# liuQuan98/GCL

Hardware: AMD Instinct MI355X
Metric: active voxels/sec thru ResUNetBN2C fwd+bwd+GCL loss, KITTI 0.3m (higher is better)
Workload: dtype f32; 1 GPU; configs[2]: GCL training step (finest_contrastive_loss), ResUNetBN2C-32 conv1 k=5, KITTI-shaped ray-cast clouds @0.3 m, bs=4 x 7 clouds per GPU, positive groups 'fixed16'; global_batch=4, parallelism=dp1

## Files before the change

gcl_amd/MinkowskiEngine/native.py:

```python
import ctypes
import os
import threading

import torch
from torch.autograd.function import once_differentiable

from .. import _lib

PLAN_ENABLED = os.environ.get("GCL_PLAN", "1") == "1"
AUX_STREAM = {"0": "", "1": "1", "low": "low", "high": "high"}[os.environ.get("GCL_PLAN_AUX", "low")]


def _addr(t):
    return t.data_ptr() if t is not None else 0


_SIDE_STREAMS = {}


def eval_side_stream(device, n_rows=None):
    if os.environ.get("GCL_EVAL_SPLIT_MAPS", "1") == "0":
        return None
    if n_rows is not None and n_rows < int(os.environ.get("GCL_EVAL_SPLIT_MIN_ROWS", "100000")):
        return None
# ... 66 lines not shown
            return None
        if addr == self.coords.data_ptr():
            return self.coords
        numel = 1
        for s in shape:
            numel *= int(s)
        nbytes = numel * torch.empty(0, dtype=dtype).element_size()
        off = addr - self.arena.data_ptr()
        if off < 0 or off + nbytes > self.arena.numel():
            raise RuntimeError("NativeMaps.view: address outside the arena")
        return self.arena[off:off + nbytes].view(dtype).view(*shape)


class _PlanRun:

    __slots__ = ("plan", "arena", "maps", "y", "x", "grad_targets", "segments", "done")

    def __del__(self):
        try:
            if not self.done and self.plan is not None and self.plan.handle and self.arena is not None:
                _lib.load().gcl_plan_release(self.plan.handle, ctypes.c_void_p(self.arena.data_ptr()))
        except Exception:
            pass


class _PlanFn(torch.autograd.Function):

    @staticmethod
    def forward(ctx, run, *params):
        ctx.run = run
        return run.y
# ... 31 lines not shown
            raise ValueError(lib.gcl_last_error().decode())
        self.handle = ctypes.c_void_p(self.handle)
        self._state = None
        self._key = None
        self.grad_targets = None
        self.bucket_of_param = None
        self.on_bucket = None
        self._param_ptrs = self._bn_ptrs = None
        self._ptr_key = None
        self.profile_next = False
        self.last_profile = None
        self._anchor = None
        self._aux = None
        self._eval_key = None
        self._touched = None

    def __del__(self):
        h, self.handle = getattr(self, "handle", None), None
        if h:
            try:
                _lib.load().gcl_plan_destroy(h)
            except Exception:
                pass

    @classmethod
    def from_tape(cls, tape, model, x_in, in_level, spec_keys):
        from . import ops
        if ops.PRECISION != "fp16x3" or not ops.FUSE_GRAD_ADD:
            raise ValueError("the plan runs the default arithmetic (fp16x3, fused gradient adds) only")
        params = [p for p in model.parameters()]
# ... 121 lines not shown
        self._ensure_state(lib, dev)
        pp, bp = self._pointers()
        if AUX_STREAM and self._aux is None:
            lo, _hi = torch.cuda.Stream.priority_range()
            pct = int(os.environ.get("GCL_AUX_CU_PCT", "0"))
            if 0 < pct < 100:
                h = ctypes.c_void_p()
                _lib.check(lib.gcl_stream_create_cu_share(pct, 1, ctypes.byref(h)), "gcl_stream_create_cu_share")
                self._aux = torch.cuda.ExternalStream(h.value, device=dev)
            else:
                self._aux = torch.cuda.Stream(device=dev, priority={"low": lo, "high": _hi}.get(AUX_STREAM, 0))
            lib.gcl_plan_set_aux_stream(self.handle, ctypes.c_void_p(self._aux.cuda_stream))
        if self.profile_next:
            lib.gcl_plan_profile(self.handle, 1)
        y_ptr = ctypes.c_void_p()
        _lib.check(lib.gcl_plan_forward(self.handle, ctypes.byref(maps.desc), _lib.ptr(x, torch.float32), pp, bp,
                                        _lib.ptr(self._state), _lib.ptr(arena), arena.numel(), ctypes.byref(y_ptr),
                                        _lib.stream()), "gcl_plan_forward")
        for m in self.bn_modules:
            m._pending_batches += 1
            m._train_forwards += 1
        n_out = int(maps.desc.n_rows[self.records[-1]["level_out"]])
        off = y_ptr.value - arena.data_ptr()
        y = arena[off:off + n_out * self.out_channels * 4].view(torch.float32).view(n_out, self.out_channels)
        if not torch.is_grad_enabled():
            lib.gcl_plan_release(self.handle, _lib.ptr(arena))
            return y
        run = _PlanRun()
        run.plan, run.arena, run.maps, run.y, run.x = self, arena, maps, y, x
        run.grad_targets, run.done = self.grad_targets, False
        run.segments = self._segments()
        if run.grad_targets is not None:
            if self._anchor is None or self._anchor.device != dev:
                self._anchor = torch.zeros(1, device=dev, requires_grad=True)
            return _PlanFn.apply(run, self._anchor)
        return _PlanFn.apply(run, *self.params)

    def _check_input(self, x_feats, maps):
        r0 = self.records[0]
        if x_feats.dim() != 2 or x_feats.shape[1] != r0["cin"]:
            raise ValueError(f"the plan was recorded for {r0['cin']} input channels, got a tensor of shape {tuple(x_feats.shape)}")
        if x_feats.shape[0] != int(maps.desc.n_rows[r0["level_in"]]):
            raise ValueError("features and coordinate maps differ in length")

    def _ensure_state(self, lib, dev):
# ... 51 lines not shown
        for i, r in enumerate(self.records):
            for k in ("w", "bias", "bn_w", "bn_b"):
                p = r[k]
                if p >= 0 and p in self.bucket_of_param:
                    b = self.bucket_of_param[p]
                    lowest[b] = min(lowest.get(b, i), i)
        cuts = sorted(set(lowest.values()), reverse=True)
        segs, hi = [], n
        for c in cuts:
            segs.append((c, hi, sorted(b for b, i in lowest.items() if i == c)))
            hi = c
        if hi > 0:
            segs.append((0, hi, []))
        return segs

    def set_touched_rows(self, rows, cap):
        lib = _lib.load()
        self._touched = rows
        _lib.check(lib.gcl_plan_set_touched_rows(self.handle, _lib.ptr(rows, torch.int32), int(cap)),
                   "gcl_plan_set_touched_rows")

    def touch_loss_rows(self, index, goff, sel, rows_a, rows_b, n_rows, cap):
        lib = _lib.load()
        dev = index.device
        scratch = torch.empty(int(lib.gcl_touched_rows_scratch_len(int(n_rows))), dtype=torch.int32, device=dev)
        out = torch.empty(int(cap) + 1, dtype=torch.int32, device=dev)
        rows, count = out[:cap], out[cap:]
        _lib.check(lib.gcl_touched_rows(_lib.ptr(index, torch.int64), index.shape[0], _lib.ptr(goff, torch.int64),
                                        goff.shape[0] - 1, _lib.ptr(sel, torch.int64), sel.shape[0],
                                        _lib.ptr(rows_a, torch.int64), rows_a.shape[0], _lib.ptr(rows_b, torch.int64),
                                        rows_b.shape[0], int(n_rows), _lib.ptr(scratch), _lib.ptr(rows), int(cap),
                                        _lib.ptr(count), _lib.stream()), "gcl_touched_rows")
        self.set_touched_rows(rows, cap)
# ... 5 lines not shown
        flat = None
        if targets is None:
            sizes = [p.numel() for p in self.params]
            flat = torch.empty(sum(sizes), dtype=torch.float32, device=dy.device)
            targets, off = [], 0
            for p, s in zip(self.params, sizes):
                targets.append(flat[off:off + s].view_as(p))
                off += s
        gp = (ctypes.c_void_p * len(targets))(*[t.data_ptr() for t in targets])
        st = _lib.stream()
        for first, last, buckets in run.segments:
            _lib.check(lib.gcl_plan_backward(self.handle, _lib.ptr(run.arena), _lib.ptr(dy, torch.float32), gp, first,
                                             last, st), "gcl_plan_backward")
            for b in buckets:
                self.on_bucket(b)
        self._touched = None
        if self.profile_next:
            self.profile_next = False
            self._profile_pending = True
            lib.gcl_plan_profile(self.handle, 0)
        run.done = True
        run.arena = run.maps = run.y = run.x = None
        return None if flat is None else targets

    def profile_records(self):
        lib = _lib.load()
        buf = (ctypes.c_double * (8 * 1024))()
        n = lib.gcl_plan_profile_read(self.handle, buf, 1024)
        return [tuple(buf[8 * i + j] for j in range(8)) for i in range(max(0, n))]
```

gcl_amd/_lib.py:

```python
import ctypes
import os
import subprocess

import torch

_HERE = os.path.dirname(os.path.abspath(__file__))
CSRC = os.path.join(_HERE, "csrc")
LIB_PATH = os.environ.get("GCL_LIB_PATH", os.path.join(CSRC, "libgcl_hip.so"))
SOURCES = ["coords.hip", "conv.hip", "norm.hip", "loss.hip", "pairloss.hip", "data.hip", "sc2pcr.hip", "plan.hip", "match.hip", "ransac.hip", "regstats.hip", "fpfh.hip",
           "valpose.hip", "pairmatch.hip", "icp.hip"]
HEADER = os.path.join(os.path.dirname(_HERE), "include", "gcl_amd.h")

_vp, _i32, _i64, _f32 = ctypes.c_void_p, ctypes.c_int32, ctypes.c_int64, ctypes.c_float
_f64 = ctypes.c_double

MAX_LEVELS, MAX_MAPS = 8, 16
MAPS_PINNED_BYTES = 512 * (MAX_MAPS + 1)
ERR_ARENA = -4


class MapSpec(ctypes.Structure):
    _fields_ = [("t_in", _i32), ("kernel_size", _i32), ("stride", _i32), ("tables", _i32), ("pairs", _i32)]


# ... 108 lines not shown
    "gcl_maps_build_split": (_i32, [_vp, _i64, _vp, _i32, _i32, _vp, _i64, _vp, _vp, _vp, _vp]),
    "gcl_plan_create": (_vp, [_vp, _i32, _i32, _i32, _vp, _i32, _i32]),
    "gcl_plan_destroy": (None, [_vp]),
    "gcl_plan_state_bytes": (_i64, [_vp]),
    "gcl_plan_arena_bytes": (_i64, [_vp, _vp]),
    "gcl_plan_forward": (_i32, [_vp, _vp, _vp, _vp, _vp, _vp, _vp, _i64, _vp, _vp]),
    "gcl_plan_eval_state_bytes": (_i64, [_vp]),
    "gcl_plan_eval_arena_bytes": (_i64, [_vp, _vp]),
    "gcl_plan_forward_eval": (_i32, [_vp, _vp, _vp, _vp, _vp, _i32, _vp, _vp, _i64, _vp, _vp]),
    "gcl_plan_backward": (_i32, [_vp, _vp, _vp, _vp, _i32, _i32, _vp]),
    "gcl_plan_release": (_i32, [_vp, _vp]),
    "gcl_plan_set_aux_stream": (_i32, [_vp, _vp]),
    "gcl_plan_touched_suffix": (_i32, [_vp]),
    "gcl_plan_set_touched_rows": (_i32, [_vp, _vp, _i64]),
    "gcl_plan_suffix_rows_used": (_i64, [_vp]),
    "gcl_gather_rows": (_i32, [_vp, _i32, _i64, _vp, _i64, _i32, _f32, _vp, _vp]),
    "gcl_scatter_rows": (_i32, [_vp, _vp, _i64, _i32, _i64, _vp, _i32, _vp]),
    "gcl_touched_rows_scratch_len": (_i64, [_i64]),
    "gcl_touched_rows": (_i32, [_vp, _i64, _vp, _i64, _vp, _i32, _vp, _i32, _vp, _i32, _i64, _vp, _vp, _i64, _vp, _vp]),
    "gcl_stream_create_cu_share": (_i32, [_i32, _i32, ctypes.POINTER(ctypes.c_void_p)]),
    "gcl_stream_destroy": (_i32, [_vp]),
    "gcl_plan_profile": (_i32, [_vp, _i32]),
    "gcl_plan_profile_read": (_i32, [_vp, _vp, _i32]),
    "gcl_sc2_chunks": (_i32, []),
    "gcl_sc2_refine_partial_len": (_i32, []),
    "gcl_sc2_confidence": (_i32, [_vp, _vp, _i32, _f32, _i32, _vp, _vp, _vp, _vp]),
    "gcl_sc2_confidence_scratch_bytes": (_i64, [_i32]),
    "gcl_sc2_confidence_sparse": (_i32, [_vp, _vp, _i32, _f32, _i32, _vp, _vp, _vp, _vp, _vp]),
    "gcl_sc2_register_scratch_bytes": (_i64, [_i32]),
    "gcl_sc2_register": (_i32, [_vp, _vp, _i32, _f32, _i32, _f32, _i32, _i32, _i32, _f32, _f32, _i32, _vp, _vp, _vp, _vp, _vp,
# ... 167 lines not shown
```

gcl_amd/csrc/plan.hip:

```cpp
#include "common.h"

#include <string.h>

#include <new>
#include <utility>
#include <vector>

namespace gcl {

__device__ __forceinline__ float amax4p(float m, const float4& v) {
  return fmaxf(m, fmaxf(fmaxf(fabsf(v.x), fabsf(v.y)), fmaxf(fabsf(v.z), fabsf(v.w))));
}
__device__ __forceinline__ void publish_amax_wg(float m, int* slot) {
#pragma unroll
  for (int o = 32; o > 0; o >>= 1) m = fmaxf(m, __shfl_xor(m, o));
  __shared__ float wm[4];
  if ((threadIdx.x & 63) == 0) wm[threadIdx.x >> 6] = m;
  __syncthreads();
  if (threadIdx.x == 0)
    amax_slot_publish(slot, __float_as_int(fmaxf(fmaxf(wm[0], wm[1]), fmaxf(wm[2], wm[3]))), blockIdx.x);
}

__global__ void __launch_bounds__(256) k_relu_fwd(const float4* __restrict__ x, long long n4, float4* __restrict__ y,
                                                  int* amax) {
// ... 94 lines not shown
    const long long j = i / cv;
    const int q = (int)(i - j * cv);
    const long long r = rows[j];
    out[i] = (r >= 0 && r < n_src) ? reinterpret_cast<const V*>(src + r * ld)[q] : splat<V>(pad);
  }
}
__global__ void __launch_bounds__(256) k_scatter_rows(const float4* __restrict__ src, const int* __restrict__ rows,
                                                      long long cap, int c4, long long n_dst, float* __restrict__ dst,
                                                      int ld) {
  const long long total = cap * c4;
  for (long long i = (long long)blockIdx.x * 256 + threadIdx.x; i < total; i += (long long)gridDim.x * 256) {
    const long long j = i / c4;
    const int q = (int)(i - j * c4);
    const long long r = rows[j];
    if (r >= 0 && r < n_dst) reinterpret_cast<float4*>(dst + r * ld)[q] = src[i];
  }
}
__global__ void __launch_bounds__(256) k_touch_rows(const long long* __restrict__ ids, long long count, long long n,
                                                    int* __restrict__ flag) {
  const long long i = (long long)blockIdx.x * 256 + threadIdx.x;
  if (i >= count) return;
  const long long r = ids[i];
  if (r >= 0 && r < n) flag[r] = 1;
}
__global__ void __launch_bounds__(64) k_touch_groups(const long long* __restrict__ index, long long n_index,
                                                     const long long* __restrict__ goff, long long n_groups,
                                                     const long long* __restrict__ sel, long long n,
                                                     int* __restrict__ flag) {
  const long long g = sel[blockIdx.x];
  if (g < 0 || g >= n_groups) return;
// ... 290 lines not shown
  std::vector<OpSaved> saved;
  std::vector<void*> params;
  Arena A{DRY_BASE, 0, 0, true};
  int32_t* slot_pool = nullptr;
  long long n_slots = 0, next_slot = 0;
  bool slots_exhausted = false;
  int32_t* w_amax = nullptr;
  unsigned char *pack_fwd = nullptr, *pack_bwd = nullptr;
  void* state = nullptr;
  bool forward_done = false, bwd_packed = false;
  std::vector<char> relu_masked;
  hipEvent_t fwd_packs = nullptr;
  bool fwd_packs_pending = false;
  int32_t* not_ones = nullptr;
  void* key = nullptr;
};

struct Plan : PassState {
  std::vector<PassState*> passes;
  std::vector<gcl_plan_op> ops;
  int n_tensors = 0, n_params = 0, n_bn = 0, presplit = 128;
  std::vector<int> worder;
  std::vector<int> widx;
  std::vector<int> wmode;
  std::vector<long long> wK, wcin, wcout, off_fwd, off_bwd;
  long long bytes_fwd = 0, bytes_bwd = 0, wgs_fwd = 0, wgs_bwd = 0;
  int n_bwd = 0;
  std::vector<char> made;
  std::vector<char> fuse_relu;
  std::vector<int> cat_left;
  std::vector<int> mask_from;
  std::vector<long long> host_tables, uploaded;
  bool eval = false;
  void* const* bn_eval = nullptr;
  bool eval_repack = true;
  hipStream_t aux = nullptr;
  std::vector<hipEvent_t> events;
  size_t events_used = 0;
  bool aux_dirty = false;
  int suffix_first = 0;
  bool suffix_rows_ok = false;
  const int32_t* touched = nullptr;
  long long touched_cap = 0;
  long long suffix_rows_used = 0;
  bool profile = false;
  std::vector<ProfRec> prof;
  size_t prof_used = 0;
};

static long long state_words(const Plan& P) { return (long long)P.worder.size() * (2 + 8 + 8); }

static int32_t* new_slot(Plan& P) {
  if (P.next_slot >= P.n_slots) {
    P.slots_exhausted = true;
    return P.slot_pool;
  }
  return P.slot_pool + (P.next_slot++) * GCL_AMAX_WORDS;
}

// ... 61 lines not shown

static bool is_stem(const gcl_plan_op& op, const gcl_map_desc& m) {
  return op.cin <= 4 && (op.cout % 32) == 0 && !op.transpose && m.kernel_size > 1 && op.bias < 0;
}

static int stem_flag(Plan& P, const gcl_plan_op& op, const gcl_map_desc& m, const TState& x, long long n_in, hipStream_t st) {
  Arena& A = P.A;
  if (!m.presence || P.not_ones) return GCL_OK;
  constexpr int CLOUD_FLAGS = 4096;
  int32_t* cloud = A.take_n<int32_t>(CLOUD_FLAGS);
  P.not_ones = A.take_n<int32_t>(n_in);
  PLAN_CALL(gcl_not_ones_rows(x.ptr, op.cin, P.maps->coords[op.level_in], n_in, cloud, CLOUD_FLAGS, P.not_ones, (void*)st));
  return GCL_OK;
}

static int conv_forward(Plan& P, int i, float** y_out, float** stats_out, hipStream_t st, int32_t** relu_amax_out) {
  Arena& A = P.A;
  const gcl_plan_op& op = P.ops[i];
  const gcl_maps_desc& M = *P.maps;
  const gcl_map_desc& m = M.maps[op.map];
  const long long n_in = M.n_rows[op.level_in], n_out = M.n_rows[op.level_out];
  TState& x = P.t[op.x];
  float* y = A.take_n<float>(n_out * op.cout);
  *y_out = y;
  *stats_out = nullptr;
  *relu_amax_out = nullptr;
  const float* W = (const float*)P.params[op.w];
  if (is_stem(op, m)) {
    int rcs = stem_flag(P, op, m, x, n_in, st);
    if (rcs) return rcs;
    PLAN_CALL(gcl_stem_fwd(x.ptr, W, m.nbr, n_out, op.K, op.cin, op.cout, y, m.presence, m.presence ? P.not_ones : nullptr,
                           (void*)st));
    return GCL_OK;
  }
  const int wi = P.widx[op.w];
  if (P.fwd_packs_pending && !A.dry) {
// ... 103 lines not shown
  }
  if (!P.eval && P.aux && P.n_bwd) {
    P.pack_bwd = (unsigned char*)A.take(P.bytes_bwd);
    if (!A.dry) {
      hipStream_t ws = fork_aux(P, st);
      const long long* tab = (const long long*)P.state;
      PLAN_CALL(gcl_pack_weights_multi((const int64_t*)(tab + 2 * nw + 8 * nw), P.n_bwd, P.wgs_bwd, 4, P.w_amax, P.pack_bwd,
                                       (void*)ws));
    }
    P.bwd_packed = true;
  }
  P.t[0].ptr = (float*)x_in;
  bool late_pending = !A.dry && M.ready_event && M.late_mask;
  for (size_t i = 0; i < P.ops.size(); ++i) {
    const gcl_plan_op& op = P.ops[i];
    const long long n_out = M.n_rows[op.level_out];
    if (late_pending && (op.kind == GCL_OP_CONVBN || op.kind == GCL_OP_CONV) && ((M.late_mask >> op.map) & 1)) {
      GCL_CHECK_HIP(hipStreamWaitEvent(st, (hipEvent_t)M.ready_event, 0));
      late_pending = false;
    }
    TState& y = P.t[op.y];
    int rc;
    switch (op.kind) {
      case GCL_OP_CONVBN: {
        if (P.eval) {
          const gcl_map_desc& m = M.maps[op.map];
          const long long n_in = M.n_rows[op.level_in];
          TState& x = P.t[op.x];
          const int c = op.cout;
          const float* res = op.x2 >= 0 ? P.t[op.x2].ptr : nullptr;
          y.ptr = A.take_n<float>(n_out * c);
// ... 69 lines not shown
          y.ld = 0;
          y.amax = bound ? bound_slot : new_slot(P);
          if (bound) y.planes = A.take(n_out * c * 4);
        }
        if (op.relu) sv.mask = A.take_n<unsigned long long>(gcl_bn_mask_len(n_out, c));
        const float* res = op.x2 >= 0 ? P.t[op.x2].ptr : nullptr;
        void* img = !bound ? nullptr : (P.cat_left[i] >= 0 ? P.t[P.ops[P.cat_left[i]].y].planes : y.planes);
        PLAN_CALL(gcl_bn_apply_planes(cy, n_out, c, sv.mean, sv.rstd, (const float*)P.params[op.bn_w],
                                      (const float*)P.params[op.bn_b], res, op.relu, y.ptr, y.ld, (uint64_t*)sv.mask, y.amax,
                                      img, (void*)st));
        break;
      }
      case GCL_OP_CONV: {
        float *cy, *stats;
        int32_t* relu_amax;
        if ((rc = conv_forward(P, (int)i, &cy, &stats, st, &relu_amax))) return rc;
        y.ptr = cy;
        if (relu_amax) {
          y.amax = relu_amax;
          P.t[P.ops[i + 1].y] = y;
        }
        break;
      }
      case GCL_OP_RELU: {
        if (i > 0 && P.fuse_relu[i - 1]) break;
        const long long n4 = n_out * op.cout / 4;
        y.ptr = A.take_n<float>(n_out * op.cout);
        y.amax = new_slot(P);
        if (!A.dry) {
          hipLaunchKernelGGL(k_relu_fwd, dim3(grid_for(n4)), dim3(256), 0, st, (const float4*)P.t[op.x].ptr, n4, (float4*)y.ptr,
                             y.amax);
          GCL_CHECK_LAUNCH();
        }
        break;
      }
      case GCL_OP_CAT: {
        const int ca = op.cin, cb = op.cout - op.cin;
        if (P.t[op.x].ld == op.cout && P.t[op.x].ptr == y.ptr && y.ptr) {
          if (!A.dry) {
            hipLaunchKernelGGL(k_cat_right, dim3(grid_for(n_out * cb / 4)), dim3(256), 0, st, (const float4*)P.t[op.x2].ptr,
// ... 15 lines not shown
        break;
      }
      case GCL_OP_ROWNORM: {
        y.ptr = A.take_n<float>(n_out * op.cout);
        P.saved[i].norm = A.take_n<float>(n_out);
        PLAN_CALL(gcl_row_normalize_fwd(P.t[op.x].ptr, n_out, op.cout, y.ptr, P.saved[i].norm, (void*)st));
        break;
      }
      default:
        set_error("gcl_plan_forward: unknown record kind %d", op.kind);
        return GCL_ERR_ARG;
    }
  }
  if (late_pending) GCL_CHECK_HIP(hipStreamWaitEvent(st, (hipEvent_t)M.ready_event, 0));
  *y_out = P.t[P.ops.back().y].ptr;
  return GCL_OK;
}

static int give(Plan& P, int tensor, float* gptr, long long numel, hipStream_t st, int32_t* amax = nullptr, int ld = 0,
                int c = 0) {
  Arena& A = P.A;
  if (tensor < 0 || !P.made[tensor] || !gptr) return GCL_OK;
  TState& g = P.g[tensor];
  if (!g.ptr) {
    g = TState();
    g.ptr = gptr;
    g.ld = ld;
    g.amax = amax;
    return GCL_OK;
  }
// ... 113 lines not shown
                                     dy.amax, scratch, dW, rgb, (void*)ws));
  }
  if (op.bias >= 0) {
    double* scratch = A.take_n<double>(gcl_bn_scratch_len(n_out, op.cout));
    PLAN_CALL(gcl_col_sum(dy.ptr, n_out, op.cout, scratch, (float*)grads[op.bias], (void*)ws));
  }
  return GCL_OK;
}

static int suffix_backward(Plan& P, const float* dy, void* const* grads, const int32_t* rows, long long cap, TState* g_out,
                           hipStream_t st) {
  Arena& A = P.A;
  const gcl_maps_desc& M = *P.maps;
  const int n_ops = (int)P.ops.size();
  const long long n = M.n_rows[P.ops.back().level_out];
  std::vector<std::pair<const float*, float*>> gathered;
  auto gather = [&](const float* src, int ld, int c, float pad) -> float* {
    for (auto& e : gathered)
      if (e.first == src) return e.second;
    float* out = A.take_n<float>(cap * c);
    if (!A.dry && gcl_gather_rows(src, ld, n, rows, cap, c, pad, out, (void*)st) != GCL_OK) return nullptr;
    gathered.push_back({src, out});
    return out;
  };
  std::vector<char> masked(P.ops.size(), 0);
  TState g;
  g.ptr = gather(dy, P.ops.back().cout, P.ops.back().cout, 0.f);
  if (!g.ptr) return GCL_ERR_ARG;
  int rc;
  for (int i = n_ops - 1; i >= P.suffix_first && g.ptr; --i) {
    const gcl_plan_op& op = P.ops[i];
    switch (op.kind) {
// ... 90 lines not shown
    P.pack_bwd = (unsigned char*)A.take(P.bytes_bwd);
    if (P.n_bwd && !A.dry) {
      const long long* tab = (const long long*)P.state;
      PLAN_CALL(gcl_pack_weights_multi((const int64_t*)(tab + 2 * nw + 8 * nw), P.n_bwd, P.wgs_bwd, 4, P.w_amax, P.pack_bwd,
                                       (void*)st));
    }
    P.bwd_packed = true;
  }
  int top = last - 1;
  long long reserve_to = 0;
  if (last == n_ops && !A.dry) P.suffix_rows_used = 0;
  if (last == n_ops && P.suffix_first < n_ops && P.suffix_rows_ok && first <= P.suffix_first) {
    const gcl_plan_op& head = P.ops[P.suffix_first];
    const long long n = M.n_rows[head.level_in];
    const long long off0 = A.off, slot0 = P.next_slot;
    if (A.dry) {
      TState g;
      const long long cap_max = (n - 1) / 2;
      if (cap_max > 0) {
        int rc = suffix_backward(P, dy, grads, nullptr, cap_max, &g, st);
        if (rc) return rc;
        A.take_n<float>(n * head.cin);
        reserve_to = A.off;
        A.off = off0;
        P.next_slot = slot0;
      }
    } else if (rows && cap > 0 && 2 * cap < n) {
      TState g;
      A.dry = true;
      int rc = suffix_backward(P, dy, grads, rows, cap, &g, st);
      A.take_n<float>(n * head.cin);
// ... 345 lines not shown
    std::vector<void*> gn(P->n_params, nullptr);
    float* yy = nullptr;
    const bool prof = P->profile;
    P->profile = false;
    rc = plan_forward(*P, x, bn_stats_host, &yy, nullptr);
    if (rc == GCL_OK) rc = plan_backward(*P, (const float*)DRY_BASE, gn.data(), 0, (int)P->ops.size(), nullptr);
    P->profile = prof;
    const long long need = P->A.off;
    P->A = real;
    if (rc) return rc;
    if (need > arena_bytes) {
      set_error("gcl_plan_forward: arena too small (%lld bytes needed, %lld given)", need, (long long)arena_bytes);
      return GCL_ERR_ARENA;
    }
  }
  rc = plan_forward(*P, x, bn_stats_host, y_out_host, (hipStream_t)stream);
  P->forward_done = rc == GCL_OK;
  if (rc != GCL_OK) return rc;
  PassState* slot = nullptr;
  for (PassState* q : P->passes)
    if (!q->forward_done || q->key == arena) slot = q;
  if (!slot) {
    slot = new (std::nothrow) PassState();
    GCL_CHECK_ARG(slot, "gcl_plan_forward: out of host memory");
    P->passes.push_back(slot);
  }
  P->key = arena;
  *slot = std::move(static_cast<PassState&>(*P));
  slot->maps = &slot->maps_copy;
  static_cast<PassState&>(*P) = PassState();
  return GCL_OK;
}

// ... 84 lines not shown
int gcl_plan_backward(void* plan, void* arena, const float* dy, void* const* grads_host, int32_t first_op,
                      int32_t last_op, void* stream) {
  Plan* P = (Plan*)plan;
  GCL_CHECK_ARG(P, "gcl_plan_backward: null pointer");
  const int32_t* rows = P->touched;
  const long long cap = P->touched_cap;
  P->touched = nullptr;
  P->touched_cap = 0;
  GCL_CHECK_ARG(grads_host, "gcl_plan_backward: null pointer");
  PassState* slot = nullptr;
  for (PassState* q : P->passes)
    if (q->forward_done && q->key == arena) slot = q;
  GCL_CHECK_ARG(slot, "gcl_plan_backward: no forward pass to differentiate in this arena");
  GCL_CHECK_ARG(first_op >= 0 && first_op < last_op && last_op <= (int)P->ops.size(), "gcl_plan_backward: bad record range");
  GCL_CHECK_ARG(last_op != (int)P->ops.size() || dy, "gcl_plan_backward: the last segment needs dy");
  static_cast<PassState&>(*P) = std::move(*slot);
  P->maps = &P->maps_copy;
  int rc = plan_backward(*P, dy, grads_host, first_op, last_op, (hipStream_t)stream, rows, cap);
  if (rc == GCL_OK && !P->A.fits()) {
    set_error("gcl_plan_backward: arena overrun");
    rc = GCL_ERR_ARENA;
  }
  if (rc == GCL_OK && P->slots_exhausted) {
    set_error("gcl_plan_backward: amax slot pool exhausted");
    rc = GCL_ERR_ARG;
  }
  if (first_op == 0 || rc != GCL_OK) P->forward_done = false;
  *slot = std::move(static_cast<PassState&>(*P));
  slot->maps = &slot->maps_copy;
  static_cast<PassState&>(*P) = PassState();
// ... 28 lines not shown

int gcl_scatter_rows(const float* src, const int32_t* rows, int64_t cap, int32_t c, int64_t n_dst, float* dst, int32_t ld,
                     void* stream) {
  GCL_CHECK_ARG(src && rows && dst && n_dst > 0 && cap > 0, "gcl_scatter_rows: bad argument");
  GCL_CHECK_ARG(c > 0 && c % 4 == 0 && ld >= c && ld % 4 == 0 && (((uintptr_t)src | (uintptr_t)dst) & 15) == 0,
                "gcl_scatter_rows: channel count and row pitch must be multiples of 4, the tensors 16-byte aligned");
  hipLaunchKernelGGL(k_scatter_rows, dim3(grid_for(cap * c / 4)), dim3(256), 0, (hipStream_t)stream, (const float4*)src,
                     (const int*)rows, (long long)cap, c / 4, (long long)n_dst, dst, ld);
  GCL_CHECK_LAUNCH();
  return GCL_OK;
}

int64_t gcl_plan_suffix_rows_used(const void* plan) {
  if (!plan) return -1;
  return ((const Plan*)plan)->suffix_rows_used;
}

int gcl_plan_set_touched_rows(void* plan, const int32_t* rows, int64_t cap) {
  Plan* P = (Plan*)plan;
  GCL_CHECK_ARG(P, "gcl_plan_set_touched_rows: null plan");
  GCL_CHECK_ARG((rows && cap > 0) || (!rows && cap == 0), "gcl_plan_set_touched_rows: a list needs a positive length");
  P->touched = rows;
  P->touched_cap = cap;
  return GCL_OK;
}

int64_t gcl_touched_rows_scratch_len(int64_t n_rows) { return n_rows > 0 ? gcl_scan_scratch_len(n_rows) : 0; }

int gcl_touched_rows(const int64_t* index, int64_t n_index, const int64_t* goff, int64_t n_groups, const int64_t* sel,
                     int32_t n_sel, const int64_t* rows_a, int32_t n_a, const int64_t* rows_b, int32_t n_b, int64_t n_rows,
// ... 74 lines not shown
```

gcl_amd/lib/colocation_trainer.py:

```python
import os
import types

import numpy as np
import torch
from torch.autograd.function import once_differentiable

import gcl_amd.MinkowskiEngine as ME
from gcl_amd import _lib
from gcl_amd.model import load_model

DEFAULT_CONFIG = dict(
    model="ResUNetBN2C", model_n_out=32, conv1_kernel_size=5, normalize_feature=True, bn_momentum=0.05,
    optimizer="SGD", lr=0.1, momentum=0.8, weight_decay=1e-4, exp_gamma=0.99,
    batch_size=4, num_pos_per_batch=256, num_hn_samples_per_batch=256, iter_size=1,
    hit_ratio_thresh=0.3, val_max_iter=400, nn_max_n=500,
    pos_thresh=0.1, neg_thresh=1.4, finest_thresh=0.2, pos_weight=1.0, neg_weight=1.0, finest_weight=1.0,
    square_loss=True, block_finest_gradient=False, use_hard_negative=True, use_pair_group_positive_loss=False,
    use_group_circle_loss=False, safe_radius=0.75, voxel_size=0.3,
    triplet_num_pos=256, triplet_num_hn=512, triplet_num_rand=1024,
)


def make_config(**overrides):
    cfg = dict(DEFAULT_CONFIG)
# ... 150 lines not shown


def prepare_loss_inputs(group, index, finest_flag, device):
    group = torch.as_tensor(group)
    goff = torch.zeros(int(group.shape[0]) + 1, dtype=torch.int64, device=device)
    goff[1:] = torch.cumsum(group.to(device, torch.int64, non_blocking=True), 0)
    index = torch.as_tensor(index).to(device, torch.int64, non_blocking=True).contiguous()
    flag = torch.as_tensor(finest_flag).to(device, non_blocking=True).to(torch.uint8).contiguous()
    return goff, index, flag


def finest_contrastive_loss(F_out, group, index, index_hash, finest_flag, max_pos_cluster=256, max_hn_samples=2048,
                            points=None, batch_lengths=None, pos_thresh=0.1, neg_thresh=1.4, finest_thresh=0.2,
                            draws=None, square_loss=True, block_finest_gradient=False,
                            use_pair_group_positive_loss=False, use_hard_negative=True, finest_term=True,
                            prepared=None, total_weights=None):
    dev = F_out.device
    n_out = F_out.shape[0]
    group = torch.as_tensor(group)
    n_groups = int(group.shape[0])
    if draws is None:
        draws = draw_selections(n_groups, n_out, max_pos_cluster, max_hn_samples,
                                group.cpu().numpy() if use_pair_group_positive_loss else None,
                                use_pair_group_positive_loss, random_negative=not use_hard_negative)
    pos_sel, sel_hn1, sel_hn2 = draws[:3]
    pair_pos = draws[3] if len(draws) > 3 else None
    rand_cols = draws[4] if len(draws) > 4 else None
    if not use_hard_negative and rand_cols is None:
        raise ValueError("use_hard_negative=False needs the drawn columns (draws[4])")
    if use_pair_group_positive_loss and pair_pos is None:
        raise ValueError("use_pair_group_positive_loss needs the drawn member positions (draws[3])")
    if len(pos_sel) == 0:
        raise ZeroDivisionError("no positive group in the batch")
    flags = (0 if square_loss else LOSS_SQRT) | (LOSS_BLOCK if block_finest_gradient else 0) | \
            (LOSS_PAIR if use_pair_group_positive_loss else 0) | (0 if finest_term else LOSS_NOFIN)
    goff, index, flag = prepared if prepared is not None else prepare_loss_inputs(group, index, finest_flag, dev)
    to_dev32 = lambda a: None if a is None else \
        torch.from_numpy(np.ascontiguousarray(a, dtype=np.int32)).to(dev, non_blocking=True)
    n_pos, n_hn = len(pos_sel), len(sel_hn1)
    sel_host = torch.empty(n_pos + 2 * n_hn, dtype=torch.int64, pin_memory=True)
    np.concatenate([np.asarray(pos_sel, dtype=np.int64), np.asarray(sel_hn1, dtype=np.int64),
                    np.asarray(sel_hn2, dtype=np.int64)], out=sel_host.numpy())
    sel_all = sel_host.to(dev, non_blocking=True)
    if total_weights is not None and use_hard_negative:
        return _GCLTotalLossFn.apply(F_out, index, goff, flag, sel_all[:n_pos], sel_all[n_pos:n_pos + n_hn],
                                     sel_all[n_pos + n_hn:], float(pos_thresh), float(finest_thresh), float(neg_thresh),
                                     flags, to_dev32(pair_pos) if use_pair_group_positive_loss else None,
                                     *[float(w) for w in total_weights])
    pos, fin, neg = _GCLLossFn.apply(F_out, index, goff, flag, sel_all[:n_pos], sel_all[n_pos:n_pos + n_hn],
                                     sel_all[n_pos + n_hn:], float(pos_thresh), float(finest_thresh), float(neg_thresh),
                                     flags, to_dev32(pair_pos) if use_pair_group_positive_loss else None)
    if not use_hard_negative:
        neg = random_negative_term(F_out, sel_all[n_pos:n_pos + n_hn], sel_all[n_pos + n_hn:], rand_cols, group, index,
                                   index_hash, float(neg_thresh))
    return pos.sum() / len(pos_sel), fin.sum() / len(pos_sel), neg


class _RandomNegFn(torch.autograd.Function):
    BLOCK_BYTES = 256 << 20

    @staticmethod
    def _blocks(m_i, m_j, c):
        rows = max(1, min(m_i, _RandomNegFn.BLOCK_BYTES // max(1, m_j * c * 4)))
        return [(a, min(m_i, a + rows)) for a in range(0, m_i, rows)]

    @staticmethod
    def _block_terms(Fi, Fj, rows_i, rows_j, n_out, pos_keys, neg_thresh):
        D = torch.sqrt(((Fi.unsqueeze(1) - Fj.unsqueeze(0)) ** 2).sum(2) + 1e-7)
        a, b = rows_j.unsqueeze(0), rows_i.unsqueeze(1)
        keys = torch.minimum(a * n_out + b, a + b * n_out)
# ... 212 lines not shown
            self._grad_views2, off = [], 0
            for p in self._params:
                self._grad_views2.append(self._flat_grad2[off:off + p.numel()].view_as(p))
                off += p.numel()
        for p, v in zip(self._params, self._grad_views):
            g = p.grad
            if g is None or g.data_ptr() != v.data_ptr():
                p.grad = v

    def _plan_buckets(self):
        if getattr(self, "_bucket_map", None) is None:
            self._bucket_map = {i: self.ddp._bucket_of[id(p)] for i, p in enumerate(self._params)}
        return self._bucket_map

    def location_loss(self, F_out, group, index, index_hash, finest_flag, max_pos_cluster, max_hn_samples,
                      points=None, batch_lengths=None, draws=None, prepared=None, total_weights=None):
        cfg = self.config
        if cfg.use_group_circle_loss:
            return location_circle_loss(F_out, group, index, index_hash, finest_flag, max_pos_cluster, max_hn_samples,
                                        points, batch_lengths, cfg.pos_thresh, cfg.neg_thresh, cfg.finest_thresh,
                                        cfg.safe_radius, 16, draws, cfg.square_loss, cfg.block_finest_gradient,
                                        cfg.use_pair_group_positive_loss)
        if cfg.finest_weight == 0:
            return location_contrastive_loss(F_out, group, index, index_hash, finest_flag, max_pos_cluster,
                                             max_hn_samples, points, batch_lengths, cfg.pos_thresh, cfg.neg_thresh,
                                             draws, cfg.use_pair_group_positive_loss, cfg.use_hard_negative)
        return finest_contrastive_loss(F_out, group, index, index_hash, finest_flag, max_pos_cluster, max_hn_samples,
                                       points, batch_lengths, cfg.pos_thresh, cfg.neg_thresh, cfg.finest_thresh, draws,
                                       cfg.square_loss, cfg.block_finest_gradient, cfg.use_pair_group_positive_loss,
                                       cfg.use_hard_negative, prepared=prepared, total_weights=total_weights)

    def forward_loss(self, input_dict, draws=None, fused_total=False):
        cfg = self.config
        sinput = ME.SparseTensor(input_dict["sinput_F"].to(self.device, non_blocking=True),
                                 coordinates=input_dict["sinput_C"].to(self.device, non_blocking=True),
                                 coordinate_manager=input_dict.get("_coordinate_manager"))
        F_out = self.model(sinput).F
        fuse = (fused_total and not cfg.use_group_circle_loss and cfg.finest_weight != 0 and cfg.use_hard_negative
                and os.environ.get("GCL_FUSED_LOSS_TOTAL", "1") == "1")
        terms = self.location_loss(
            F_out, input_dict["group"], input_dict["index"], input_dict.get("index_hash"), input_dict["finest_flag"],
            max_pos_cluster=cfg.num_pos_per_batch * cfg.batch_size,
            max_hn_samples=cfg.num_hn_samples_per_batch * cfg.batch_size,
            points=input_dict["sinput_C"][:, 1:] if cfg.use_group_circle_loss else None,
            batch_lengths=input_dict.get("batch_lengths"), draws=draws, prepared=input_dict.get("_loss_inputs"),
            total_weights=(self.pos_weight, self.finest_weight, self.neg_weight) if fuse else None)
        if len(terms) == 4:
            return terms[0], tuple(terms[1:]), F_out
        pos, fin, neg = terms
        loss = self.pos_weight * pos + self.finest_weight * fin + self.neg_weight * neg
        return loss, (pos, fin, neg), F_out

    def _touched_cap(self, input_dict, draws):
        if self.config.use_group_circle_loss or draws is None:
            return None
        sizes = input_dict.get("_group_host", input_dict["group"])
        if isinstance(sizes, torch.Tensor):
            if sizes.is_cuda:
                return None
            sizes = sizes.numpy()
        pos_sel, sel_hn1, sel_hn2 = draws[:3]
        cap = int(np.asarray(sizes)[np.asarray(pos_sel)].sum()) + len(sel_hn1) + len(sel_hn2)
        return (cap + 127) // 128 * 128

    def _draw_for(self, input_dict):
        cfg = self.config
        if cfg.use_group_circle_loss:
            sizes = torch.as_tensor(input_dict["group"]).cpu().numpy() if cfg.use_pair_group_positive_loss else None
            return draw_circle_selections(len(input_dict["group"]), cfg.num_pos_per_batch * cfg.batch_size, sizes,
                                          cfg.use_pair_group_positive_loss)
        sizes = None
        if cfg.use_pair_group_positive_loss:
            sizes = torch.as_tensor(input_dict["group"]).cpu().numpy()
        return draw_selections(len(input_dict["group"]), len(input_dict["sinput_C"]),
                               cfg.num_pos_per_batch * cfg.batch_size, cfg.num_hn_samples_per_batch * cfg.batch_size,
                               sizes, cfg.use_pair_group_positive_loss, random_negative=not cfg.use_hard_negative)

    def _prefetch_maps(self, batch):
# ... 209 lines not shown
                    p.grad = None
            else:
                self.optimizer.zero_grad(set_to_none=False)
        tot_loss, tot_parts, n_rows = None, None, 0
        for i, (b, d) in enumerate(zip(micro, mdraws)):
            if self.ddp is not None:
                self.ddp.set_last_microstep(i == n_micro - 1)
            if plan is not None:
                plan.grad_targets = self._grad_views if i == 0 else self._grad_views2
                overlap = self.ddp is not None and n_micro == 1 and self.ddp.overlap and self.ddp.world > 1
                plan.bucket_of_param = self._plan_buckets() if overlap else None
                plan.on_bucket = self.ddp.bucket_ready if overlap else None
            wait_for_batch(b)
            try:
                cap = self._touched_cap(b, d) if plan is not None else None
                _TOUCHED_REQUEST = (plan, cap) if cap else None
                loss, parts, F_out = self.forward_loss(b, d, fused_total=(n_micro == 1))
                _TOUCHED_REQUEST = None
                if n_micro > 1:
                    parts = tuple(p / n_micro for p in parts)
                    loss = self.pos_weight * parts[0] + self.finest_weight * parts[1] + self.neg_weight * parts[2]
                loss.backward()
            finally:
                _TOUCHED_REQUEST = None
                if plan is not None:
                    plan.set_touched_rows(None, 0)
                    plan.grad_targets = plan.bucket_of_param = plan.on_bucket = None
            if plan is not None and i > 0:
                self._flat_grad.add_(self._flat_grad2)
            release_batch(b)
            n_rows += F_out.shape[0]
            dl, dp = loss.detach(), tuple(p.detach() for p in parts)
# ... 76 lines not shown
```

include/gcl_amd.h:

```cpp
#ifndef GCL_AMD_H
#define GCL_AMD_H

#include <stdint.h>

#ifdef __cplusplus
extern "C" {
#endif

#define GCL_OK 0
#define GCL_ERR_ARG (-1)
#define GCL_ERR_HIP (-2)
#define GCL_ERR_NO_DEVICE (-3)

#define GCL_PAIR_CHUNK 128

const char* gcl_last_error(void);
int gcl_version(void);
int gcl_device_count(void);

int gcl_coords_insert(const int32_t* coords, int64_t n, int64_t* table, int64_t cap,
                      int32_t* status, void* stream);

int64_t gcl_scan_scratch_len(int64_t n);
int gcl_stride_map(const int32_t* coords_in, int64_t n_in, const int32_t* n_in_dev, int32_t t_out,
// ... 360 lines not shown
int gcl_plan_forward(void* plan, const gcl_maps_desc* maps_host, const float* x, void* const* params_host,
                     void* const* bn_stats_host, void* state, void* arena, int64_t arena_bytes, float** y_out_host,
                     void* stream);
int64_t gcl_plan_eval_state_bytes(const void* plan);
int64_t gcl_plan_eval_arena_bytes(void* plan, const gcl_maps_desc* maps_host);
int gcl_plan_forward_eval(void* plan, const gcl_maps_desc* maps_host, const float* x, void* const* params_host,
                          void* const* bn_eval_host, int32_t repack, void* state, void* arena, int64_t arena_bytes,
                          float** y_out_host, void* stream);
int gcl_plan_backward(void* plan, void* arena, const float* dy, void* const* grads_host, int32_t first_op,
                      int32_t last_op, void* stream);
int gcl_plan_release(void* plan, void* arena);
int gcl_plan_set_aux_stream(void* plan, void* stream);
int gcl_plan_touched_suffix(const void* plan);
int gcl_plan_set_touched_rows(void* plan, const int32_t* rows, int64_t cap);
int64_t gcl_plan_suffix_rows_used(const void* plan);
int64_t gcl_touched_rows_scratch_len(int64_t n_rows);
int gcl_touched_rows(const int64_t* index, int64_t n_index, const int64_t* goff, int64_t n_groups, const int64_t* sel,
                     int32_t n_sel, const int64_t* rows_a, int32_t n_a, const int64_t* rows_b, int32_t n_b, int64_t n_rows,
                     int32_t* scratch, int32_t* rows, int64_t cap, int32_t* n_touched, void* stream);
int gcl_gather_rows(const float* src, int32_t ld, int64_t n_src, const int32_t* rows, int64_t cap, int32_t c, float pad,
                    float* out, void* stream);
int gcl_scatter_rows(const float* src, const int32_t* rows, int64_t cap, int32_t c, int64_t n_dst, float* dst, int32_t ld,
                     void* stream);
int gcl_stream_create_cu_share(int32_t percent, int32_t low_priority, void** stream_out);
int gcl_stream_destroy(void* stream);
int gcl_plan_profile(void* plan, int32_t enable);
int gcl_plan_profile_read(void* plan, double* records_host, int32_t max_records);

int gcl_col_sum(const float* x, int64_t n, int32_t c, double* scratch, float* out, void* stream);

// ... 57 lines not shown
```

Before: 46.89 million active voxels/s.

## Run the network's tail forward only on rows the loss touches

Before the forward pass, the trainer now works out which output rows the GCL loss will read and hands that list to the plan. The plan gathers those rows at the head of the final pointwise suffix and runs the suffix forward on the compact set only. It then scatters the results into a zeroed dense output, marking untouched rows of a row-norm output as inert. Backward reuses the compact suffix tensors instead of gathering again. This removes dense suffix compute and memory traffic over rows the loss never reads, at the cost of a dry-run sizing pass, extra gather/scatter and memset kernels, and a constraint that backward segments must not cut the suffix.

```diff
diff --git a/gcl_amd/MinkowskiEngine/native.py b/gcl_amd/MinkowskiEngine/native.py
--- a/gcl_amd/MinkowskiEngine/native.py
+++ b/gcl_amd/MinkowskiEngine/native.py
@@ -104,7 +104,7 @@
 
 class _PlanRun:
 
-    __slots__ = ("plan", "arena", "maps", "y", "x", "grad_targets", "segments", "done")
+    __slots__ = ("plan", "arena", "maps", "y", "x", "grad_targets", "segments", "done", "touched")
 
     def __del__(self):
         try:
@@ -166,6 +166,7 @@
         self._aux = None
         self._eval_key = None
         self._touched = None
+        self._touched_cap = 0
 
     def __del__(self):
         h, self.handle = getattr(self, "handle", None), None
@@ -317,9 +318,17 @@
         if self.profile_next:
             lib.gcl_plan_profile(self.handle, 1)
         y_ptr = ctypes.c_void_p()
-        _lib.check(lib.gcl_plan_forward(self.handle, ctypes.byref(maps.desc), _lib.ptr(x, torch.float32), pp, bp,
-                                        _lib.ptr(self._state), _lib.ptr(arena), arena.numel(), ctypes.byref(y_ptr),
-                                        _lib.stream()), "gcl_plan_forward")
+        held = None
+        if self._touched is not None and not (torch.is_grad_enabled() and self.forward_list_ok()):
+            held, cap = self._touched, self._touched_cap
+            self.set_touched_rows(None, 0)
+        try:
+            _lib.check(lib.gcl_plan_forward(self.handle, ctypes.byref(maps.desc), _lib.ptr(x, torch.float32), pp, bp,
+                                            _lib.ptr(self._state), _lib.ptr(arena), arena.numel(), ctypes.byref(y_ptr),
+                                            _lib.stream()), "gcl_plan_forward")
+        finally:
+            if held is not None:
+                self.set_touched_rows(held, cap)
         for m in self.bn_modules:
             m._pending_batches += 1
             m._train_forwards += 1
@@ -332,6 +341,9 @@
         run = _PlanRun()
         run.plan, run.arena, run.maps, run.y, run.x = self, arena, maps, y, x
         run.grad_targets, run.done = self.grad_targets, False
+        run.touched = None
+        if self._touched is not None and lib.gcl_plan_suffix_fwd_rows_used(self.handle) > 0:
+            run.touched, self._touched, self._touched_cap = self._touched, None, 0
         run.segments = self._segments()
         if run.grad_targets is not None:
             if self._anchor is None or self._anchor.device != dev:
@@ -413,9 +425,17 @@
             segs.append((0, hi, []))
         return segs
 
+    def forward_list_ok(self):
+        n, s = len(self.records), _lib.load().gcl_plan_touched_suffix(self.handle)
+        return all(last <= s or (first <= s and last == n) for first, last, _ in self._segments())
+
+    def output_rows(self, maps):
+        return int(maps.desc.n_rows[self.records[-1]["level_out"]])
+
     def set_touched_rows(self, rows, cap):
         lib = _lib.load()
         self._touched = rows
+        self._touched_cap = int(cap)
         _lib.check(lib.gcl_plan_set_touched_rows(self.handle, _lib.ptr(rows, torch.int32), int(cap)),
                    "gcl_plan_set_touched_rows")
 
@@ -451,7 +471,7 @@
                                              last, st), "gcl_plan_backward")
             for b in buckets:
                 self.on_bucket(b)
-        self._touched = None
+        self._touched = run.touched = None
         if self.profile_next:
             self.profile_next = False
             self._profile_pending = True
diff --git a/gcl_amd/_lib.py b/gcl_amd/_lib.py
--- a/gcl_amd/_lib.py
+++ b/gcl_amd/_lib.py
@@ -146,6 +146,7 @@
     "gcl_plan_touched_suffix": (_i32, [_vp]),
     "gcl_plan_set_touched_rows": (_i32, [_vp, _vp, _i64]),
     "gcl_plan_suffix_rows_used": (_i64, [_vp]),
+    "gcl_plan_suffix_fwd_rows_used": (_i64, [_vp]),
     "gcl_gather_rows": (_i32, [_vp, _i32, _i64, _vp, _i64, _i32, _f32, _vp, _vp]),
     "gcl_scatter_rows": (_i32, [_vp, _vp, _i64, _i32, _i64, _vp, _i32, _vp]),
     "gcl_touched_rows_scratch_len": (_i64, [_i64]),
diff --git a/gcl_amd/csrc/plan.hip b/gcl_amd/csrc/plan.hip
--- a/gcl_amd/csrc/plan.hip
+++ b/gcl_amd/csrc/plan.hip
@@ -132,6 +132,22 @@
     const int q = (int)(i - j * c4);
     const long long r = rows[j];
     if (r >= 0 && r < n_dst) reinterpret_cast<float4*>(dst + r * ld)[q] = src[i];
+  }
+}
+__global__ void __launch_bounds__(256) k_scatter_rows_inert(float4* __restrict__ y, float* __restrict__ norm,
+                                                            const int* __restrict__ rows, long long cap, int c4,
+                                                            long long n_dst, float* __restrict__ dst, int ld) {
+  const long long total = cap * c4;
+  for (long long i = (long long)blockIdx.x * 256 + threadIdx.x; i < total; i += (long long)gridDim.x * 256) {
+    const long long j = i / c4;
+    const int q = (int)(i - j * c4);
+    const long long r = rows[j];
+    if (r >= 0 && r < n_dst) {
+      reinterpret_cast<float4*>(dst + r * ld)[q] = y[i];
+    } else {
+      y[i] = make_float4(0.f, 0.f, 0.f, 0.f);
+      if (q == 0) norm[j] = 1.f;
+    }
   }
 }
 __global__ void __launch_bounds__(256) k_touch_rows(const long long* __restrict__ ids, long long count, long long n,
@@ -452,6 +468,8 @@
   bool fwd_packs_pending = false;
   int32_t* not_ones = nullptr;
   void* key = nullptr;
+  const int32_t* fwd_rows = nullptr;
+  long long fwd_cap = 0;
 };
 
 struct Plan : PassState {
@@ -481,6 +499,7 @@
   const int32_t* touched = nullptr;
   long long touched_cap = 0;
   long long suffix_rows_used = 0;
+  long long suffix_fwd_rows_used = 0;
   bool profile = false;
   std::vector<ProfRec> prof;
   size_t prof_used = 0;
@@ -572,12 +591,13 @@
   return GCL_OK;
 }
 
-static int conv_forward(Plan& P, int i, float** y_out, float** stats_out, hipStream_t st, int32_t** relu_amax_out) {
+static int conv_forward(Plan& P, int i, float** y_out, float** stats_out, hipStream_t st, int32_t** relu_amax_out,
+                        long long rows = 0) {
   Arena& A = P.A;
   const gcl_plan_op& op = P.ops[i];
   const gcl_maps_desc& M = *P.maps;
   const gcl_map_desc& m = M.maps[op.map];
-  const long long n_in = M.n_rows[op.level_in], n_out = M.n_rows[op.level_out];
+  const long long n_in = rows > 0 ? rows : M.n_rows[op.level_in], n_out = rows > 0 ? rows : M.n_rows[op.level_out];
   TState& x = P.t[op.x];
   float* y = A.take_n<float>(n_out * op.cout);
   *y_out = y;
@@ -711,7 +731,18 @@
   bool late_pending = !A.dry && M.ready_event && M.late_mask;
   for (size_t i = 0; i < P.ops.size(); ++i) {
     const gcl_plan_op& op = P.ops[i];
-    const long long n_out = M.n_rows[op.level_out];
+    const bool compact = P.fwd_cap > 0 && (int)i >= P.suffix_first;
+    const long long n_out = compact ? P.fwd_cap : M.n_rows[op.level_out];
+    if (compact && (int)i == P.suffix_first) {
+      TState& xs = P.t[op.x];
+      float* cx = A.take_n<float>(P.fwd_cap * op.cin);
+      PLAN_CALL(gcl_gather_rows(xs.ptr, xs.ld ? xs.ld : op.cin, M.n_rows[op.level_in], P.fwd_rows, P.fwd_cap, op.cin, 0.f, cx,
+                                (void*)st));
+      int32_t* slot = xs.amax;
+      xs = TState();
+      xs.ptr = cx;
+      xs.amax = slot;
+    }
     if (late_pending && (op.kind == GCL_OP_CONVBN || op.kind == GCL_OP_CONV) && ((M.late_mask >> op.map) & 1)) {
       GCL_CHECK_HIP(hipStreamWaitEvent(st, (hipEvent_t)M.ready_event, 0));
       late_pending = false;
@@ -811,7 +842,7 @@
       case GCL_OP_CONV: {
         float *cy, *stats;
         int32_t* relu_amax;
-        if ((rc = conv_forward(P, (int)i, &cy, &stats, st, &relu_amax))) return rc;
+        if ((rc = conv_forward(P, (int)i, &cy, &stats, st, &relu_amax, compact ? P.fwd_cap : 0))) return rc;
         y.ptr = cy;
         if (relu_amax) {
           y.amax = relu_amax;
@@ -820,7 +851,10 @@
         break;
       }
       case GCL_OP_RELU: {
-        if (i > 0 && P.fuse_relu[i - 1]) break;
+        if (i > 0 && P.fuse_relu[i - 1]) {
+          if (compact) y = P.t[op.x];
+          break;
+        }
         const long long n4 = n_out * op.cout / 4;
         y.ptr = A.take_n<float>(n_out * op.cout);
         y.amax = new_slot(P);
@@ -866,6 +900,24 @@
   }
   if (late_pending) GCL_CHECK_HIP(hipStreamWaitEvent(st, (hipEvent_t)M.ready_event, 0));
   *y_out = P.t[P.ops.back().y].ptr;
+  if (P.fwd_cap > 0) {
+    const gcl_plan_op& last = P.ops.back();
+    const long long n = M.n_rows[last.level_out];
+    float* yc = *y_out;
+    float* out = A.take_n<float>(n * last.cout);
+    if (!A.dry) {
+      GCL_CHECK_HIP(hipMemsetAsync(out, 0, (size_t)(n * last.cout) * sizeof(float), st));
+      if (last.kind == GCL_OP_ROWNORM) {
+        hipLaunchKernelGGL(k_scatter_rows_inert, dim3(grid_for(P.fwd_cap * last.cout / 4)), dim3(256), 0, st, (float4*)yc,
+                           P.saved[P.ops.size() - 1].norm, (const int*)P.fwd_rows, P.fwd_cap, last.cout / 4, n, out, last.cout);
+        GCL_CHECK_LAUNCH();
+      } else {
+        int rc = gcl_scatter_rows(yc, P.fwd_rows, P.fwd_cap, last.cout, n, out, last.cout, (void*)st);
+        if (rc) return rc;
+      }
+    }
+    *y_out = out;
+  }
   return GCL_OK;
 }
 
@@ -1009,8 +1061,10 @@
   const gcl_maps_desc& M = *P.maps;
   const int n_ops = (int)P.ops.size();
   const long long n = M.n_rows[P.ops.back().level_out];
+  const bool parked = P.fwd_cap > 0;
   std::vector<std::pair<const float*, float*>> gathered;
   auto gather = [&](const float* src, int ld, int c, float pad) -> float* {
+    if (parked && src != dy) return (float*)src;
     for (auto& e : gathered)
       if (e.first == src) return e.second;
     float* out = A.take_n<float>(cap * c);
@@ -1131,7 +1185,22 @@
     const gcl_plan_op& head = P.ops[P.suffix_first];
     const long long n = M.n_rows[head.level_in];
     const long long off0 = A.off, slot0 = P.next_slot;
-    if (A.dry) {
+    if (P.fwd_cap > 0) {
+      TState g;
+      int rc = suffix_backward(P, dy, grads, P.fwd_rows, P.fwd_cap, &g, st);
+      if (rc) return rc;
+      P.g[P.ops.back().y] = TState();
+      if (g.ptr) {
+        float* dx = A.take_n<float>(n * head.cin);
+        if (!A.dry) {
+          GCL_CHECK_HIP(hipMemsetAsync(dx, 0, (size_t)(n * head.cin) * sizeof(float), st));
+          if ((rc = gcl_scatter_rows(g.ptr, P.fwd_rows, P.fwd_cap, head.cin, n, dx, head.cin, (void*)st))) return rc;
+        }
+        if ((rc = give(P, head.x, dx, n * head.cin, st, g.amax, 0, head.cin))) return rc;
+      }
+      top = P.suffix_first - 1;
+      if (!A.dry) P.suffix_rows_used = P.fwd_cap;
+    } else if (A.dry) {
       TState g;
       const long long cap_max = (n - 1) / 2;
       if (cap_max > 0) {
@@ -1507,9 +1576,39 @@
       return GCL_ERR_ARENA;
     }
   }
+  const int n_ops = (int)P->ops.size();
+  P->suffix_fwd_rows_used = 0;
+  if (P->touched && P->touched_cap > 0 && P->suffix_first < n_ops && P->suffix_rows_ok && P->ops.back().cout % 4 == 0 &&
+      2 * P->touched_cap < maps_host->n_rows[P->ops[P->suffix_first].level_in]) {
+    Arena real = P->A;
+    P->A = Arena{DRY_BASE, 0, 0, true};
+    P->fwd_rows = P->touched;
+    P->fwd_cap = P->touched_cap;
+    std::vector<void*> gn(P->n_params, nullptr);
+    float* yy = nullptr;
+    const bool prof = P->profile;
+    P->profile = false;
+    rc = plan_forward(*P, x, bn_stats_host, &yy, nullptr);
+    if (rc == GCL_OK) rc = plan_backward(*P, (const float*)DRY_BASE, gn.data(), 0, n_ops, nullptr);
+    P->profile = prof;
+    if (rc != GCL_OK || P->A.off > arena_bytes) {
+      P->fwd_rows = nullptr;
+      P->fwd_cap = 0;
+    }
+    P->A = real;
+  }
   rc = plan_forward(*P, x, bn_stats_host, y_out_host, (hipStream_t)stream);
   P->forward_done = rc == GCL_OK;
-  if (rc != GCL_OK) return rc;
+  if (rc != GCL_OK) {
+    P->fwd_rows = nullptr;
+    P->fwd_cap = 0;
+    return rc;
+  }
+  if (P->fwd_cap > 0) {
+    P->suffix_fwd_rows_used = P->fwd_cap;
+    P->touched = nullptr;
+    P->touched_cap = 0;
+  }
   PassState* slot = nullptr;
   for (PassState* q : P->passes)
     if (!q->forward_done || q->key == arena) slot = q;
@@ -1624,6 +1723,14 @@
   GCL_CHECK_ARG(slot, "gcl_plan_backward: no forward pass to differentiate in this arena");
   GCL_CHECK_ARG(first_op >= 0 && first_op < last_op && last_op <= (int)P->ops.size(), "gcl_plan_backward: bad record range");
   GCL_CHECK_ARG(last_op != (int)P->ops.size() || dy, "gcl_plan_backward: the last segment needs dy");
+  if (slot->fwd_cap > 0) {
+    GCL_CHECK_ARG(!rows || (rows == slot->fwd_rows && cap == slot->fwd_cap),
+                  "gcl_plan_backward: the forward pass of this arena ran the touched-row suffix on another list");
+    GCL_CHECK_ARG(last_op <= P->suffix_first || (first_op <= P->suffix_first && last_op == (int)P->ops.size()),
+                  "gcl_plan_backward: the record range [%d, %d) cuts the touched-row suffix [%d, %d), which the forward pass "
+                  "ran on the rows of a list: there are no dense operands to fall back to",
+                  (int)first_op, (int)last_op, P->suffix_first, (int)P->ops.size());
+  }
   static_cast<PassState&>(*P) = std::move(*slot);
   P->maps = &P->maps_copy;
   int rc = plan_backward(*P, dy, grads_host, first_op, last_op, (hipStream_t)stream, rows, cap);
@@ -1682,6 +1789,11 @@
 int64_t gcl_plan_suffix_rows_used(const void* plan) {
   if (!plan) return -1;
   return ((const Plan*)plan)->suffix_rows_used;
+}
+
+int64_t gcl_plan_suffix_fwd_rows_used(const void* plan) {
+  if (!plan) return -1;
+  return ((const Plan*)plan)->suffix_fwd_rows_used;
 }
 
 int gcl_plan_set_touched_rows(void* plan, const int32_t* rows, int64_t cap) {
diff --git a/gcl_amd/lib/colocation_trainer.py b/gcl_amd/lib/colocation_trainer.py
--- a/gcl_amd/lib/colocation_trainer.py
+++ b/gcl_amd/lib/colocation_trainer.py
@@ -188,7 +188,7 @@
                             points=None, batch_lengths=None, pos_thresh=0.1, neg_thresh=1.4, finest_thresh=0.2,
                             draws=None, square_loss=True, block_finest_gradient=False,
                             use_pair_group_positive_loss=False, use_hard_negative=True, finest_term=True,
-                            prepared=None, total_weights=None):
+                            prepared=None, total_weights=None, selections=None):
     dev = F_out.device
     n_out = F_out.shape[0]
     group = torch.as_tensor(group)
@@ -212,10 +212,7 @@
     to_dev32 = lambda a: None if a is None else \
         torch.from_numpy(np.ascontiguousarray(a, dtype=np.int32)).to(dev, non_blocking=True)
     n_pos, n_hn = len(pos_sel), len(sel_hn1)
-    sel_host = torch.empty(n_pos + 2 * n_hn, dtype=torch.int64, pin_memory=True)
-    np.concatenate([np.asarray(pos_sel, dtype=np.int64), np.asarray(sel_hn1, dtype=np.int64),
-                    np.asarray(sel_hn2, dtype=np.int64)], out=sel_host.numpy())
-    sel_all = sel_host.to(dev, non_blocking=True)
+    sel_all = selections if selections is not None else upload_selections(pos_sel, sel_hn1, sel_hn2, dev)
     if total_weights is not None and use_hard_negative:
         return _GCLTotalLossFn.apply(F_out, index, goff, flag, sel_all[:n_pos], sel_all[n_pos:n_pos + n_hn],
                                      sel_all[n_pos + n_hn:], float(pos_thresh), float(finest_thresh), float(neg_thresh),
@@ -228,6 +225,14 @@
         neg = random_negative_term(F_out, sel_all[n_pos:n_pos + n_hn], sel_all[n_pos + n_hn:], rand_cols, group, index,
                                    index_hash, float(neg_thresh))
     return pos.sum() / len(pos_sel), fin.sum() / len(pos_sel), neg
+
+
+def upload_selections(pos_sel, sel_hn1, sel_hn2, dev):
+    n_pos, n_hn = len(pos_sel), len(sel_hn1)
+    sel_host = torch.empty(n_pos + 2 * n_hn, dtype=torch.int64, pin_memory=True)
+    np.concatenate([np.asarray(pos_sel, dtype=np.int64), np.asarray(sel_hn1, dtype=np.int64),
+                    np.asarray(sel_hn2, dtype=np.int64)], out=sel_host.numpy())
+    return sel_host.to(dev, non_blocking=True)
 
 
 class _RandomNegFn(torch.autograd.Function):
@@ -470,7 +475,7 @@
         return self._bucket_map
 
     def location_loss(self, F_out, group, index, index_hash, finest_flag, max_pos_cluster, max_hn_samples,
-                      points=None, batch_lengths=None, draws=None, prepared=None, total_weights=None):
+                      points=None, batch_lengths=None, draws=None, prepared=None, total_weights=None, selections=None):
         cfg = self.config
         if cfg.use_group_circle_loss:
             return location_circle_loss(F_out, group, index, index_hash, finest_flag, max_pos_cluster, max_hn_samples,
@@ -484,9 +489,10 @@
         return finest_contrastive_loss(F_out, group, index, index_hash, finest_flag, max_pos_cluster, max_hn_samples,
                                        points, batch_lengths, cfg.pos_thresh, cfg.neg_thresh, cfg.finest_thresh, draws,
                                        cfg.square_loss, cfg.block_finest_gradient, cfg.use_pair_group_positive_loss,
-                                       cfg.use_hard_negative, prepared=prepared, total_weights=total_weights)
-
-    def forward_loss(self, input_dict, draws=None, fused_total=False):
+                                       cfg.use_hard_negative, prepared=prepared, total_weights=total_weights,
+                                       selections=selections)
+
+    def forward_loss(self, input_dict, draws=None, fused_total=False, selections=None):
         cfg = self.config
         sinput = ME.SparseTensor(input_dict["sinput_F"].to(self.device, non_blocking=True),
                                  coordinates=input_dict["sinput_C"].to(self.device, non_blocking=True),
@@ -500,7 +506,7 @@
             max_hn_samples=cfg.num_hn_samples_per_batch * cfg.batch_size,
             points=input_dict["sinput_C"][:, 1:] if cfg.use_group_circle_loss else None,
             batch_lengths=input_dict.get("batch_lengths"), draws=draws, prepared=input_dict.get("_loss_inputs"),
-            total_weights=(self.pos_weight, self.finest_weight, self.neg_weight) if fuse else None)
+            total_weights=(self.pos_weight, self.finest_weight, self.neg_weight) if fuse else None, selections=selections)
         if len(terms) == 4:
             return terms[0], tuple(terms[1:]), F_out
         pos, fin, neg = terms
@@ -518,6 +524,21 @@
         pos_sel, sel_hn1, sel_hn2 = draws[:3]
         cap = int(np.asarray(sizes)[np.asarray(pos_sel)].sum()) + len(sel_hn1) + len(sel_hn2)
         return (cap + 127) // 128 * 128
+
+    def _touch_forward(self, plan, input_dict, draws, cap):
+        prep, mgr = input_dict.get("_loss_inputs"), input_dict.get("_coordinate_manager")
+        maps = getattr(mgr, "native", None)
+        if prep is None or maps is None or self.config.finest_weight == 0 or not plan.forward_list_ok():
+            return None
+        n_rows = plan.output_rows(maps)
+        if 2 * cap >= n_rows:
+            return None
+        pos_sel, sel_hn1, sel_hn2 = draws[:3]
+        n_pos, n_hn = len(pos_sel), len(sel_hn1)
+        sel_all = upload_selections(pos_sel, sel_hn1, sel_hn2, self.device)
+        goff, index, _ = prep
+        plan.touch_loss_rows(index, goff, sel_all[:n_pos], sel_all[n_pos:n_pos + n_hn], sel_all[n_pos + n_hn:], n_rows, cap)
+        return sel_all
 
     def _draw_for(self, input_dict):
         cfg = self.config
@@ -757,8 +778,9 @@
             wait_for_batch(b)
             try:
                 cap = self._touched_cap(b, d) if plan is not None else None
-                _TOUCHED_REQUEST = (plan, cap) if cap else None
-                loss, parts, F_out = self.forward_loss(b, d, fused_total=(n_micro == 1))
+                sel_dev = self._touch_forward(plan, b, d, cap) if cap else None
+                _TOUCHED_REQUEST = (plan, cap) if cap and sel_dev is None else None
+                loss, parts, F_out = self.forward_loss(b, d, fused_total=(n_micro == 1), selections=sel_dev)
                 _TOUCHED_REQUEST = None
                 if n_micro > 1:
                     parts = tuple(p / n_micro for p in parts)
diff --git a/include/gcl_amd.h b/include/gcl_amd.h
--- a/include/gcl_amd.h
+++ b/include/gcl_amd.h
@@ -398,6 +398,7 @@
 int gcl_plan_touched_suffix(const void* plan);
 int gcl_plan_set_touched_rows(void* plan, const int32_t* rows, int64_t cap);
 int64_t gcl_plan_suffix_rows_used(const void* plan);
+int64_t gcl_plan_suffix_fwd_rows_used(const void* plan);
 int64_t gcl_touched_rows_scratch_len(int64_t n_rows);
 int gcl_touched_rows(const int64_t* index, int64_t n_index, const int64_t* goff, int64_t n_groups, const int64_t* sel,
                      int32_t n_sel, const int64_t* rows_a, int32_t n_a, const int64_t* rows_b, int32_t n_b, int64_t n_rows,
```

Measured after the change: 47.44 million active voxels/s, median of 6. +1.2%, better.
